# arneschneuing/DiffSBDD

Hardware: AMD Instinct MI355X
Metric: sampled ligands/sec (500-step DDPM, fullatom_cond) at 1/2/4/8 MI355X (higher is better)
Workload: dtype f32

## Files before the change

diffsbdd_amd/csrc/engine.hip:

```cpp
#include "../../include/diffsbdd_hip.h"

#include <cstdio>
#include <cstdlib>
#include <cstring>
#include <string>
#include <vector>

#include "common.h"
#include "ddpm.h"
#include "edge_mlp.h"
#include "edge_wave.h"
#include "edge_wave16.h"
#include "edge_splitk.h"
#include "graph.h"
#include "lig_head.h"
#include "molecule.h"
#include "node_chain.h"
#include "node_linear.h"
#include "train.h"

using namespace dsbdd;

static thread_local std::string g_err;
static int fail(int code, const std::string& msg) { g_err = msg; return code; }

#define HIP_TRY(expr)                                                              \
  do {                                                                             \
    hipError_t _e = (expr);                                                        \
    if (_e != hipSuccess)                                                          \
      return fail(DSBDD_ERR_LAUNCH, std::string(#expr) + ": " + hipGetErrorString(_e)); \
  } while (0)

struct StreamDevice {
  int prev = -1;
  bool switched = false;
  explicit StreamDevice(void* stream) {
    hipStream_t s = static_cast<hipStream_t>(stream);
    if (!s) return;
    hipDevice_t d = 0;
    int cur = 0;
    if (hipStreamGetDevice(s, &d) != hipSuccess || hipGetDevice(&cur) != hipSuccess) { (void)hipGetLastError(); return; }
    if ((int)d != cur) { prev = cur; switched = hipSetDevice((int)d) == hipSuccess; }
  }
  ~StreamDevice() { if (switched) (void)hipSetDevice(prev); }
  StreamDevice(const StreamDevice&) = delete;
  StreamDevice& operator=(const StreamDevice&) = delete;
};

static inline int pad4(int v) { return (v + 3) & ~3; }
static inline size_t al256(size_t v) { return (v + 255) & ~(size_t)255; }

struct dsbdd_engine {
  dsbdd_config cfg;
  std::vector<const float*> slots;
  bool has_weights = false;
  char* ws = nullptr;
  size_t ws_bytes = 0;
  int64_t cap_lig = 0, cap_poc = 0, cap_batch = 0, cap_edges = 0;
  int *node_batch, *lig_off, *poc_off, *deg, *row_ptr, *erow, *ecol;
  int *act_flag, *act_ptr, *act_list;
  float *ed0, *x, *x_in, *xagg, *mean, *h0, *enc_tmp, *h, *t1, *agg, *pq, *pqg, *hout, *w2tp;
  float *agg_head, *xagg_head;
  int *scan_tmp, *seg_base, *tile_ctr;
  int *erow2, *ecol2, *row_ptr2, *deg2, *scan_tmp2, *seg_base2;
  int *erow3, *ecol3, *row_ptr3, *deg3, *scan_tmp3, *seg_base3, *node_batch3, *lig_off3, *poc_off3, *twin;
  float *ed02, *ed03, *xframe, *aggB, *agg_headB;
  int* frame_rows;
  int *lvl, *seg_rows, *seg_edges, *node_base, *edge_base, *lvl_cnt, *lvl_end, *lvl_list, *row_ptrL, *erowL, *ecolL;
  float* ed0L;
  unsigned long long* lvl_stats = nullptr;
  bool lvl_stats_zeroed = false;
  int64_t cap_edgesL = 0;
  int prune = 1;
  int cone = 1;
  int64_t ghost_slots = 0;
  std::vector<int> plan_radius, plan_ghost;
  int plan_timed_level = kLevels - 1;
  bool frame = false;
  int64_t frame_nlig = 0, frame_npoc = 0, frame_batch = 0, frame_n3 = 0, frame_cap3 = 0;
  bool ghost_dirty = true;
  bool h0_pocket_valid = false;
  int64_t cap_tiles = 0;
  int64_t cap_tiles16 = 0;
  unsigned granule16 = 0;
  bool w2tp16_ready = false;
  unsigned splitk = 0;
  bool w2sk_ready = false;
  int emu = 0;
  bool w2e_ready = false;
  float *trace_h = nullptr, *trace_x = nullptr;
  int n_cu = 256;
  bool w2tp_ready = false;
  float* wchain = nullptr;
  bool wchain_ready = false;
  int chain = 1;
  int64_t chain_min_rows = 0;
  int fork_front = 0;
  hipStream_t side_stream = nullptr;
  hipEvent_t ev_fork = nullptr, ev_join = nullptr;
  int level_rows = 0;
  int fold_scan = 1;
  int lig_head = 1;
  int edge_bperm = 1;
  int profile = 0;
  int64_t prof_call = 0;
  bool time_now = false;
  std::vector<hipEvent_t> ev;
  size_t ev_used = 0;
  struct GraphEntry {
    std::vector<uint64_t> key;
    int seen = 0;
    hipGraph_t graph = nullptr;
    hipGraphExec_t exec = nullptr;
    std::vector<int> plan_radius, plan_ghost;
    int plan_timed_level = 0;
  };
  std::vector<GraphEntry> graphs;
  int use_graph = 1;
  int coord_split = 1;
  int node_group = 1;
  int edge_max_wg = 0;
  int64_t n_replay = 0, n_capture = 0, n_eager = 0;
  unsigned long long* ts_buf = nullptr;
  int ts_cap = 0, ts_next = 0;
  hipStream_t cap_stream = nullptr;
  void drop_graphs() {
    for (GraphEntry& g : graphs) {
      if (g.exec) (void)hipGraphExecDestroy(g.exec);
      if (g.graph) (void)hipGraphDestroy(g.graph);
    }
    graphs.clear();
  }
  ~dsbdd_engine() {
    for (hipEvent_t e : ev) (void)hipEventDestroy(e);
    drop_graphs();
    if (cap_stream) (void)hipStreamDestroy(cap_stream);
    if (side_stream) (void)hipStreamDestroy(side_stream);
    if (ev_fork) (void)hipEventDestroy(ev_fork);
    if (ev_join) (void)hipEventDestroy(ev_join);
  }
};

static int n_slots(const dsbdd_config& c) {
  return DSBDD_G_COUNT + c.n_layers * (c.inv_sublayers * DSBDD_GCL_COUNT + DSBDD_EQ_COUNT);
}
static int gcl_slot(const dsbdd_config& c, int block, int sub, int which) {
  return DSBDD_G_COUNT + block * (c.inv_sublayers * DSBDD_GCL_COUNT + DSBDD_EQ_COUNT) +
         sub * DSBDD_GCL_COUNT + which;
}
static int eq_slot(const dsbdd_config& c, int block, int which) {
  return DSBDD_G_COUNT + block * (c.inv_sublayers * DSBDD_GCL_COUNT + DSBDD_EQ_COUNT) +
         c.inv_sublayers * DSBDD_GCL_COUNT + which;
}

struct WsLayout {
  size_t off[72];
  size_t total;
};

static WsLayout carve(const dsbdd_config& c, int64_t nl, int64_t np, int64_t B, int64_t E) {
  const int64_t N = nl + np;
  const int H = c.hidden_nf, JP = pad4(c.joint_nf + 1);
  const int LE = pad4(2 * (c.atom_nf > c.residue_nf ? c.atom_nf : c.residue_nf));
  const int PQ = (c.reflection_equivariant ? 2 : 4) * H;
  const int64_t EL = 2 * E + 32 * kLevels * B;
  const int64_t NG = N + np;
  const int64_t T = EL / 32 + 2;
  size_t sizes[] = {
      (size_t)N * 4, (size_t)(B + 1) * 4, (size_t)(B + 1) * 4, (size_t)NG * 4, (size_t)(N + 1) * 4,
      (size_t)E * 4, (size_t)E * 4, (size_t)E * 4,
      (size_t)NG * 12, (size_t)N * 12, (size_t)N * 24, (size_t)B * 12,
      (size_t)N * JP * 4, (size_t)N * LE * 4,
      (size_t)NG * H * 4, (size_t)NG * H * 4, (size_t)NG * H * 4, (size_t)N * PQ * 4,
      (size_t)N * JP * 4,
      (size_t)N * 4, (size_t)(N + 1) * 4, (size_t)N * 4,
      (size_t)NG * 2 * H * 4,
      (size_t)c.n_layers * (c.inv_sublayers + 2) * H * H * 18 + 4096,
      (size_t)2 * T * H * 4, (size_t)2 * T * 2 * 16,
      (size_t)(N + 1) * 4, (size_t)(2 * B + 1) * 4, (size_t)kTileCtrInts * 4,
      (size_t)E * 4, (size_t)E * 4, (size_t)E * 4, (size_t)(N + 1) * 4, (size_t)N * 4,
      (size_t)(N + 1) * 4, (size_t)(2 * B + 1) * 4,
      (size_t)E * 4, (size_t)E * 4, (size_t)E * 4, (size_t)(N + 1) * 4, (size_t)N * 4,
      (size_t)(N + 1) * 4, (size_t)(2 * B + 1) * 4,
      (size_t)N * 4, (size_t)(B + 1) * 4, (size_t)(B + 1) * 4, (size_t)N * 4,
      (size_t)N * 12, (size_t)NG * H * 4, (size_t)T * H * 4,
      (size_t)N * 4, (size_t)kLevels * B * 4, (size_t)kLevels * B * 4,
      (size_t)(kLevels * B + 1) * 4, (size_t)(kLevels * B + 1) * 4, 64, 64,
      (size_t)NG * 4, (size_t)(NG + 1) * 4, (size_t)EL * 4, (size_t)EL * 4, (size_t)EL * 4,
      128, (size_t)N * 4,
      (size_t)c.n_layers * ((size_t)c.inv_sublayers * 5 * H * H + (size_t)H * PQ) * 4 + 4096};
  WsLayout L;
  size_t o = 0;
  const int n = sizeof(sizes) / sizeof(sizes[0]);
  for (int i = 0; i < n; ++i) { L.off[i] = o; o += al256(sizes[i] + 16); }
  L.total = o;
  return L;
}

static int build_edges_impl(hipStream_t s, const float* x, int n_lig, int N, int B, const dsbdd_config& c,
                            const int* node_batch, const int* lig_off, const int* poc_off, int* deg,
                            int* row_ptr, int* erow, int* ecol, float* ed0, int64_t cap, int* status,
                            int* act_flag = nullptr, int* scan_tmp = nullptr, int* seg_base = nullptr,
                            const EdgeList2* list2 = nullptr, int id_offset = 0, int* lvl = nullptr);

extern "C" {

int dsbdd_abi_version(void) { return DSBDD_ABI_VERSION; }
const char* dsbdd_last_error(void) { return g_err.c_str(); }

int dsbdd_engine_create(const dsbdd_config* cfg, dsbdd_engine** out) {
  if (!cfg || !out) return fail(DSBDD_ERR_ARG, "null argument");
  const int H = cfg->hidden_nf;
  if (!(H == 64 || H == 128 || H == 192 || H == 256))
    return fail(DSBDD_ERR_ARG, "hidden_nf must be one of 64, 128, 192, 256");
  if (cfg->n_layers < 1 || cfg->inv_sublayers < 1 || cfg->atom_nf < 1 || cfg->residue_nf < 1 ||
      cfg->joint_nf < 1 || cfg->edge_embedding_dim < 0)
    return fail(DSBDD_ERR_ARG, "bad layer/feature counts");
  if (!(cfg->normalization_factor > 0.f)) return fail(DSBDD_ERR_ARG, "normalization_factor must be > 0");
  dsbdd_engine* e = new dsbdd_engine();
  e->cfg = *cfg;
  e->slots.assign(n_slots(*cfg), nullptr);
  int dev = 0;
  hipDeviceProp_t prop;
  if (hipGetDevice(&dev) == hipSuccess && hipGetDeviceProperties(&prop, dev) == hipSuccess &&
      prop.multiProcessorCount > 0)
    e->n_cu = prop.multiProcessorCount;
  const char* ug = getenv("DSBDD_GRAPH");
  if (ug && atoi(ug) == 0) e->use_graph = 0;
  const char* bpe = getenv("DSBDD_EDGE_BPERM");
  if (bpe && atoi(bpe) == 0) e->edge_bperm = 0;
  const char* csp = getenv("DSBDD_COORD_SPLIT");
  if (csp && atoi(csp) == 0) e->coord_split = 0;
  const char* ngp = getenv("DSBDD_NODE_GROUP");
  if (ngp && atoi(ngp) == 0) e->node_group = 0;
  const char* prn = getenv("DSBDD_PRUNE");
  if (prn && atoi(prn) == 0) e->prune = 0;
  if (const char* lh = getenv("DSBDD_LIG_HEAD")) e->lig_head = atoi(lh) != 0;
  if (const char* fs = getenv("DSBDD_FOLD_SCAN")) e->fold_scan = atoi(fs) > 0 ? 1 : 0;
  if (const char* lr = getenv("DSBDD_LEVEL_ROWS")) e->level_rows = atoi(lr) != 0;
  if (const char* fk = getenv("DSBDD_FORK")) e->fork_front = atoi(fk) != 0;
  if (const char* g16 = getenv("DSBDD_GRANULE16")) e->granule16 = (unsigned)strtoul(g16, nullptr, 0);
  if (const char* sk = getenv("DSBDD_SPLITK")) e->splitk = (unsigned)strtoul(sk, nullptr, 0);
  if (const char* em = getenv("DSBDD_EMU")) { const int v = atoi(em); e->emu = (v == 6 || v == 9) ? v : 0; }
  const char* cn = getenv("DSBDD_CONE");
  if (cn) e->cone = atoi(cn) <= 0 ? 0 : (atoi(cn) >= 2 ? 2 : 1);
  const char* nch = getenv("DSBDD_NODE_CHAIN");
  if (nch && atoi(nch) == 0) e->chain = 0;
  const char* ncm = getenv("DSBDD_NODE_CHAIN_MIN_ROWS");
  if (ncm && atoi(ncm) >= 0) e->chain_min_rows = atoi(ncm);
  const char* mwg = getenv("DSBDD_EDGE_MAX_WG");
  if (mwg && atoi(mwg) > 0) e->edge_max_wg = atoi(mwg);
  *out = e;
  return DSBDD_OK;
}

void dsbdd_engine_destroy(dsbdd_engine* e) { delete e; }

int dsbdd_engine_weight_slots(const dsbdd_engine* e) { return e ? n_slots(e->cfg) : DSBDD_ERR_ARG; }

int dsbdd_engine_set_weights(dsbdd_engine* e, const float* const* slots_host, int n) {
  if (!e || !slots_host) return fail(DSBDD_ERR_ARG, "null argument");
  if (n != n_slots(e->cfg)) return fail(DSBDD_ERR_ARG, "wrong number of weight slots");
  const dsbdd_config& c = e->cfg;
  for (int i = 0; i < n; ++i) {
    const float* ptr = slots_host[i];
    bool optional = false;
    const int per = c.inv_sublayers * DSBDD_GCL_COUNT + DSBDD_EQ_COUNT;
    if (i >= DSBDD_G_COUNT) {
      const int r = (i - DSBDD_G_COUNT) % per;
      if (r < c.inv_sublayers * DSBDD_GCL_COUNT) {
        const int wch = r % DSBDD_GCL_COUNT;
        if (!c.attention && (wch == DSBDD_GCL_ATT_W || wch == DSBDD_GCL_ATT_B)) optional = true;
      } else {
        const int wch = r - c.inv_sublayers * DSBDD_GCL_COUNT;
        if (c.reflection_equivariant && wch >= DSBDD_EQ_X_WD && wch <= DSBDD_EQ_X_B2) optional = true;
      }
    }
    if (!ptr && !optional) return fail(DSBDD_ERR_ARG, "null weight slot " + std::to_string(i));
    if (ptr && (reinterpret_cast<uintptr_t>(ptr) & 15))
      return fail(DSBDD_ERR_ARG, "weight slot " + std::to_string(i) + " not 16-byte aligned");
    e->slots[i] = ptr;
  }
  e->drop_graphs();
  e->w2tp_ready = false;
  e->w2tp16_ready = false;
  e->w2sk_ready = false;
  e->w2e_ready = false;
  e->wchain_ready = false;
  e->h0_pocket_valid = false;
  e->has_weights = true;
  return DSBDD_OK;
}

size_t dsbdd_engine_workspace_bytes(const dsbdd_engine* e, int64_t nl, int64_t np, int64_t B,
                                    int64_t E) {
  if (!e || nl < 0 || np < 0 || B < 1 || E < 0) return 0;
  return carve(e->cfg, nl, np, B, E).total;
}

int dsbdd_engine_bind_workspace(dsbdd_engine* e, void* ws, size_t bytes, int64_t nl, int64_t np,
                                int64_t B, int64_t E) {
  if (!e || !ws) return fail(DSBDD_ERR_ARG, "null argument");
  if (reinterpret_cast<uintptr_t>(ws) & 255) return fail(DSBDD_ERR_ARG, "workspace must be 256-byte aligned");
  if ((nl + np) >= (1ll << 30) || E >= (1ll << 31) - 256) return fail(DSBDD_ERR_ARG, "problem too large for int32 indices");
  WsLayout L = carve(e->cfg, nl, np, B, E);
  if (bytes < L.total) return fail(DSBDD_ERR_CAPACITY, "workspace too small");
  char* b = static_cast<char*>(ws);
  e->drop_graphs();
  e->ws = b; e->ws_bytes = bytes;
  e->cap_lig = nl; e->cap_poc = np; e->cap_batch = B; e->cap_edges = E;
  e->node_batch = (int*)(b + L.off[0]); e->lig_off = (int*)(b + L.off[1]); e->poc_off = (int*)(b + L.off[2]);
  e->deg = (int*)(b + L.off[3]); e->row_ptr = (int*)(b + L.off[4]);
  e->erow = (int*)(b + L.off[5]); e->ecol = (int*)(b + L.off[6]); e->ed0 = (float*)(b + L.off[7]);
  e->x = (float*)(b + L.off[8]); e->x_in = (float*)(b + L.off[9]); e->xagg = (float*)(b + L.off[10]);
  e->mean = (float*)(b + L.off[11]); e->h0 = (float*)(b + L.off[12]); e->enc_tmp = (float*)(b + L.off[13]);
  e->h = (float*)(b + L.off[14]); e->t1 = (float*)(b + L.off[15]); e->agg = (float*)(b + L.off[16]);
  e->pq = (float*)(b + L.off[17]); e->hout = (float*)(b + L.off[18]);
  e->act_flag = (int*)(b + L.off[19]); e->act_ptr = (int*)(b + L.off[20]); e->act_list = (int*)(b + L.off[21]);
  e->pqg = (float*)(b + L.off[22]);
  e->w2tp = (float*)(b + L.off[23]);
// ... 548 lines not shown
    return (e->splitk && can_sk) ? reinterpret_cast<const float*>(reinterpret_cast<const char*>(e->w2tp) + n_w2 * H * H * 14) +
                                       ((size_t)blk * (c.inv_sublayers + 2) + which) * H * H
                                 : nullptr;
  };
  if (e->splitk && can_sk && !e->w2sk_ready) {
    for (int blk = 0; blk < c.n_layers; ++blk)
      for (int which = 0; which < c.inv_sublayers + 2; ++which) {
        const float* src = which < c.inv_sublayers ? W[gcl_slot(c, blk, which, DSBDD_GCL_E2_WT)]
                         : W[eq_slot(c, blk, which == c.inv_sublayers ? DSBDD_EQ_C_W2T : DSBDD_EQ_X_W2T)];
        if (!src) continue;
        hipLaunchKernelGGL(pack_w2sk_kernel, dim3((H * H + 255) / 256), dim3(256), 0, s, src,
                           const_cast<float*>(w2sk_of(blk, which)), H);
        HIP_TRY(hipGetLastError());
      }
    e->w2sk_ready = true;
  }
  if (e->emu && !e->w2e_ready) {
    for (int blk = 0; blk < c.n_layers; ++blk)
      for (int which = 0; which < c.inv_sublayers + 2; ++which) {
        const float* src = which < c.inv_sublayers ? W[gcl_slot(c, blk, which, DSBDD_GCL_E2_WT)]
                         : W[eq_slot(c, blk, which == c.inv_sublayers ? DSBDD_EQ_C_W2T : DSBDD_EQ_X_W2T)];
        if (!src) continue;
        hipLaunchKernelGGL(pack_w2e_kernel, dim3((H * H + 255) / 256), dim3(256), 0, s, src,
                           reinterpret_cast<unsigned short*>(const_cast<void*>(w2e_of(blk, which))), H);
        HIP_TRY(hipGetLastError());
      }
    e->w2e_ready = true;
  }
  if (e->granule16 && !e->w2tp16_ready) {
    for (int blk = 0; blk < c.n_layers; ++blk)
      for (int which = 0; which < c.inv_sublayers + 2; ++which) {
        const float* src = which < c.inv_sublayers ? W[gcl_slot(c, blk, which, DSBDD_GCL_E2_WT)]
                         : W[eq_slot(c, blk, which == c.inv_sublayers ? DSBDD_EQ_C_W2T : DSBDD_EQ_X_W2T)];
        if (!src) continue;
        hipLaunchKernelGGL(pack16_w2t_kernel, dim3((H * H + 255) / 256), dim3(256), 0, s, src,
                           const_cast<float*>(w2tp16_of(blk, which)), H);
        HIP_TRY(hipGetLastError());
      }
    e->w2tp16_ready = true;
  }
  if (bperm && !e->w2tp_ready) {
    for (int blk = 0; blk < c.n_layers; ++blk)
      for (int which = 0; which < c.inv_sublayers + 2; ++which) {
        const float* src = which < c.inv_sublayers ? W[gcl_slot(c, blk, which, DSBDD_GCL_E2_WT)]
                         : W[eq_slot(c, blk, which == c.inv_sublayers ? DSBDD_EQ_C_W2T : DSBDD_EQ_X_W2T)];
        if (!src) continue;
        hipLaunchKernelGGL(permute_w2t_kernel, dim3((H * H + 255) / 256), dim3(256), 0, s, src,
                           const_cast<float*>(w2tp_of(blk, which)), H);
        HIP_TRY(hipGetLastError());
      }
    e->w2tp_ready = true;
  }
  const bool use_chain = e->chain && (H == 256 || H == 192 || H == 128) && N >= e->chain_min_rows;
  const size_t chain_blk = (size_t)c.inv_sublayers * 5 * H * H + (size_t)H * PQ;
  auto chain_w = [&](int blk, int sub, int which) -> const float* {
    const float* base = e->wchain + (size_t)blk * chain_blk;
    if (which == 3) return base + (size_t)c.inv_sublayers * 5 * H * H;
    return base + (size_t)sub * 5 * H * H + (which == 0 ? 0 : (which == 1 ? 2 * H * H : 3 * H * H));
  };
  if (use_chain && !e->wchain_ready) {
    auto pack = [&](const float* WT, int ldw, int K, int Ncols, const float* dst) {
      hipLaunchKernelGGL(pack_b16_kernel, dim3((K * Ncols + 255) / 256), dim3(256), 0, s, WT, ldw, K, Ncols,
                         const_cast<float*>(dst));
    };
    for (int blk = 0; blk < c.n_layers; ++blk) {
      for (int sub = 0; sub < c.inv_sublayers; ++sub) {
        pack(W[gcl_slot(c, blk, sub, DSBDD_GCL_N1_WT)], H, 2 * H, H, chain_w(blk, sub, 0));
        pack(W[gcl_slot(c, blk, sub, DSBDD_GCL_N2_WT)], H, H, H, chain_w(blk, sub, 1));
        pack(W[gcl_slot(c, blk, sub, DSBDD_GCL_E1_WT)], 2 * H, H, 2 * H, chain_w(blk, sub, 2));
      }
      pack(W[eq_slot(c, blk, DSBDD_EQ_C1_WT)], PQ, H, PQ, chain_w(blk, 0, 3));
    }
    HIP_TRY(hipGetLastError());
    e->wchain_ready = true;
  }
  auto gcl_pq = [&](int blk, int sub) {
    NodeLinearArgs a{e->h, H, H, nullptr, 0, 0, W[gcl_slot(c, blk, sub, DSBDD_GCL_E1_WT)], 2 * H, nullptr,
                     nullptr, 0, e->pqg, 2 * H, (int)N, 2 * H, 0, nullptr, nullptr};
    const int g = blk * c.inv_sublayers + sub;
    rows_of(radius_of(g) + 1, g <= g_ghost_last && g > 0, a);
    return a;
  };
  bool pqg_ready = false, chained_pq = false, chained_coord = false;
  for (int blk = 0; blk < c.n_layers; ++blk) {
    if (n_mlp == 2 && (blk == 0 || !subset) && !(blk == 0 && mean_in_levels)) {
      hipLaunchKernelGGL(sample_mean_kernel, dim3(B), dim3(kThreads), 0, s, (const float*)e->x,
                         (const int*)e->lig_off, (const int*)e->poc_off, nlig, e->mean);
      HIP_TRY(hipGetLastError());
    }
    for (int sub = 0; sub < c.inv_sublayers; ++sub) {
      auto G = [&](int which) { return W[gcl_slot(c, blk, sub, which)]; };
      if (sub > 0 && chained_pq) pqg_ready = true;
      if (!pqg_ready) {
        const bool rows0 = split0 && blk == 0 && sub == 0;
        NodeLinearArgs grp0[2];
        if (rows0) {
          grp0[0] = gcl_pq(blk, sub);
          grp0[0].row_idx = act_rows; grp0[0].m_count = act_count; grp0[0].M = N;
          grp0[1] = gcl_pq(blk, sub);
          grp0[1].A1 = e->h + (size_t)N * H; grp0[1].C = e->pqg + (size_t)N * 2 * H; grp0[1].M = n_frame_rows;
          grp0[1].row_idx = nullptr; grp0[1].m_count = nullptr;
        }
        if (!(rows0 && launch_node_group(s, grp0, 2) == hipSuccess)) {
          (void)hipGetLastError();
          HIP_TRY(launch_node_linear(s, gcl_pq(blk, sub)));
          if (rows0) HIP_TRY(launch_node_linear(s, grp0[1]));
        }
      }
      pqg_ready = false;
      const int g = blk * c.inv_sublayers + sub;
      const int radius = radius_of(g);
      const bool ghost = g <= g_ghost_last;
      const bool all_rows = !prune || radius >= LV;
      const int64_t begin = ghost ? 0 : ghost_slots;
      EdgeArgs ea{};
      ea.erow = L_row + begin; ea.ecol = L_col + begin; ea.ed0 = L_d0 + begin;
      ea.e_count = !prune ? e_all : (ghost ? e->lvl_end + radius : e->lvl_end + kLevels + radius);
      ea.e_cap = L_cap - (int)begin; ea.wt_base = (int)(begin / 32); ea.x = e->x;
      ea.n_lig = nlig; ea.n_nodes = N + n_frame_rows; ea.ldpq = 2 * H;
      ea.mlp[0] = EdgeMlpW{e->pqg, e->pqg + H, G(DSBDD_GCL_E1_WD), G(DSBDD_GCL_E1_WD0), G(DSBDD_GCL_E1_TAB),
                           G(DSBDD_GCL_E2_WT), G(DSBDD_GCL_E2_B), w2tp_of(blk, sub), w2tp16_of(blk, sub), w2e_of(blk, sub),
                           w2sk_of(blk, sub)};
      ea.mlp[1] = ea.mlp[0];
      const bool g16 = ((e->granule16 >> (g & 15)) & 1u) && !(split0 && blk == 0 && sub == 0) && !e->emu;
      const bool gsk = ((e->splitk >> (g & 15)) & 1u) && can_sk;
      ea.att_w = G(DSBDD_GCL_ATT_W); ea.att_b = G(DSBDD_GCL_ATT_B); ea.attention = c.attention;
      ea.agg = e->agg; ea.agg_head = e->agg_head; ea.tile_ctr = e->tile_ctr;
      ea.norm_factor = c.normalization_factor;
      if (split0 && blk == 0 && sub == 0) {
        EdgeArgs a2 = ea;
        a2.erow = e->erow2; a2.ecol = e->ecol2; a2.ed0 = e->ed02; a2.e_count = e->row_ptr2 + N;
        a2.e_cap = (int)e->cap_edges; a2.wt_base = 0;
        EdgeArgs a3 = ea;
        a3.erow = e->erow3; a3.ecol = e->ecol3; a3.ed0 = e->ed03; a3.e_count = e->row_ptr3 + e->frame_n3;
        a3.agg = e->aggB; a3.agg_head = e->agg_headB; a3.e_cap = (int)e->cap_edges; a3.wt_base = 0;
        a2.erow_b = a3.erow; a2.ecol_b = a3.ecol; a2.ed0_b = a3.ed0; a2.e_count_b = a3.e_count; a2.e_cap_b = a3.e_cap;
        a2.wt_base_b = a3.wt_base; a2.agg_b = a3.agg; a2.agg_head_b = a3.agg_head;
        HIP_TRY(launch_edge(e, s, MODE_GCL, a2, edge_bound + ((e->frame_cap3 + 127) / 128) * 128, false, gsk));
        hipLaunchKernelGGL(agg_complete2_kernel, dim3((N + n_ghost + 3) / 4), dim3(kThreads), 0, s, e->agg,
                           (const float*)e->agg_head, (const int*)e->row_ptr2, (const int*)e->deg2,
                           (const float*)e->aggB, (const float*)e->agg_headB, (const int*)e->row_ptr3,
                           (const int*)e->deg3, (const int*)e->twin, N, nlig, N, H, cone ? n_ghost : 0, (int)e->cap_tiles - 1);
        HIP_TRY(hipGetLastError());
      } else {
        const bool timed = e->time_now && (all_rows || radius == e->plan_timed_level) && e->ev_used + 2 <= e->ev.size();
        if (timed) HIP_TRY(hipEventRecord(e->ev[e->ev_used], s));
        HIP_TRY(launch_edge(e, s, MODE_GCL, ea, L_bound, g16 && !gsk, gsk));
        if (timed) {
          HIP_TRY(hipEventRecord(e->ev[e->ev_used + 1], s));
          e->ev_used += 2;
        }
        const int n_rows = N + (ghost ? n_ghost : 0);
        hipLaunchKernelGGL(agg_complete_kernel, dim3((n_rows + 3) / 4), dim3(kThreads), 0, s, e->agg,
                           (const float*)e->agg_head, L_ptr, (const int*)e->deg, n_rows, H,
                           (int)((g16 && !gsk) ? e->cap_tiles16 : e->cap_tiles) - 1, (g16 && !gsk) ? 4 : 5);
        HIP_TRY(hipGetLastError());
      }
      NodeLinearArgs n1{e->h, H, H, e->agg, H, H, G(DSBDD_GCL_N1_WT), H, G(DSBDD_GCL_N1_B), nullptr, 0, e->t1, H,
                        (int)N, H, 1, nullptr, nullptr};
      NodeLinearArgs n2{e->t1, H, H, nullptr, 0, 0, G(DSBDD_GCL_N2_WT), H, G(DSBDD_GCL_N2_B), e->h, H, e->h, H,
                        (int)N, H, 0, nullptr, nullptr};
      rows_of(radius, ghost, n1); rows_of(radius, ghost, n2);
      chained_pq = false; chained_coord = false;
      bool fill_pq = false;
      if (use_chain) {
        NodeChainArgs ca{};
        ca.row_idx = n1.row_idx; ca.m_count = n1.m_count; ca.M = n1.M; ca.do_mlp = 1;
        ca.h = e->h; ca.agg = e->agg;
        ca.W1p = chain_w(blk, sub, 0); ca.b1 = G(DSBDD_GCL_N1_B);
        ca.W2p = chain_w(blk, sub, 1); ca.b2 = G(DSBDD_GCL_N2_B);
        const bool last_sub = sub + 1 == c.inv_sublayers;
        const int first = ghost ? n_ghost : 0;
        if (last_sub) {
          const int QW = n_mlp * H;
          const float* wc = chain_w(blk, 0, 3);
          if (!subset) {
            ca.proj[ca.n_proj++] = ChainProj{wc, e->pq, PQ, PQ, nullptr, 0};
            chained_coord = true;
          } else if (prune && n1.row_idx) {
            ca.proj[ca.n_proj++] = ChainProj{wc, e->pq, PQ, QW, act_count, first};
            ca.proj[ca.n_proj++] = ChainProj{wc + (size_t)(QW / 16) * (H / 16) * 256, e->pq + QW, PQ, QW,
                                             e->lvl_cnt + kLevels, first};
            chained_coord = true;
          }
        }
        const bool has_next = !last_sub || blk + 1 < c.n_layers;
        if (has_next) {
          const int nb = last_sub ? blk + 1 : blk, ns = last_sub ? 0 : sub + 1;
          const NodeLinearArgs nx = gcl_pq(nb, ns);
          const bool same_rows = nx.row_idx == n1.row_idx && nx.m_count == n1.m_count && nx.M == n1.M;
          if (same_rows || ghost) {
            ca.proj[ca.n_proj++] = ChainProj{chain_w(nb, ns, 2), e->pqg, 2 * H, 2 * H, nullptr, 0};
            chained_pq = true;
            fill_pq = ghost && !same_rows;
          }
        }
        HIP_TRY(launch_node_chain(s, ca, H, e->n_cu));
      } else {
        HIP_TRY(launch_node_linear(s, n1));
        HIP_TRY(launch_node_linear(s, n2));
      }
      if (ghost) {
        const int hi = radius_of(g + 1) + 1 < LV ? radius_of(g + 1) + 1 : LV;
        if (hi > radius) {
          hipLaunchKernelGGL(canon_fill_kernel, dim3((N - nlig + 3) / 4), dim3(kThreads), 0, s, e->h,
                             (const int*)e->lvl, (const int*)e->twin, nlig, N, N, radius, hi, H,
                             fill_pq ? e->pqg : (float*)nullptr, 2 * H);
          fill_pq = false;
          HIP_TRY(hipGetLastError());
        }
      }
    }
    {
      auto Q = [&](int which) { return W[eq_slot(c, blk, which)]; };
      const int QW = n_mlp * H;
      NodeLinearArgs grp[kMaxGroup];
      int ng = 0;
      if (!chained_coord) {
        if (subset) {
          grp[ng++] = NodeLinearArgs{e->h, H, H, nullptr, 0, 0, Q(DSBDD_EQ_C1_WT), PQ, nullptr, nullptr, 0, e->pq, PQ,
                                     (int)N, QW, 0, act_rows, act_count};
          grp[ng++] = NodeLinearArgs{e->h, H, H, nullptr, 0, 0, Q(DSBDD_EQ_C1_WT) + QW, PQ, nullptr, nullptr, 0,
                                     e->pq + QW, PQ, (int)n_lig, QW, 0, nullptr, nullptr};
        } else {
          grp[ng++] = NodeLinearArgs{e->h, H, H, nullptr, 0, 0, Q(DSBDD_EQ_C1_WT), PQ, nullptr, nullptr, 0, e->pq, PQ,
                                     (int)N, PQ, 0, nullptr, nullptr};
        }
      }
      const int n_coord = ng;
      const bool want_next = blk + 1 < c.n_layers && !chained_pq;
      if (chained_pq && blk + 1 < c.n_layers) pqg_ready = true;
      if (want_next && use_chain) {
        const NodeLinearArgs nx = gcl_pq(blk + 1, 0);
        NodeChainArgs ca{};
        ca.row_idx = nx.row_idx; ca.m_count = nx.m_count; ca.M = nx.M; ca.do_mlp = 0; ca.h = e->h;
        ca.n_proj = 1;
        ca.proj[0] = ChainProj{chain_w(blk + 1, 0, 2), e->pqg, 2 * H, 2 * H, nullptr, 0};
        HIP_TRY(launch_node_chain(s, ca, H, e->n_cu));
        pqg_ready = true;
      } else if (want_next) {
        grp[ng++] = gcl_pq(blk + 1, 0);
      }
      if (ng > 0) {
        if (e->node_group && launch_node_group(s, grp, ng) == hipSuccess) {
          if (ng > n_coord) pqg_ready = true;
        } else {
          (void)hipGetLastError();
          for (int i = 0; i < n_coord; ++i) HIP_TRY(launch_node_linear(s, grp[i]));
        }
      }
      chained_pq = false;
// ... 945 lines not shown
```

diffsbdd_amd/csrc/node_chain.h:

```cpp
#pragma once
#include "common.h"

namespace dsbdd {

typedef float f32x4 __attribute__((ext_vector_type(4)));

#ifdef DSBDD_CHAIN_TS
__device__ unsigned long long* g_chain_ts = nullptr;
__device__ __forceinline__ void chain_ts(int slot) {
  if (g_chain_ts && threadIdx.x == 0 && slot < 16) {
    g_chain_ts[blockIdx.x * 32 + slot] = __builtin_readcyclecounter();
    g_chain_ts[blockIdx.x * 32 + 16 + slot] = wall_clock64();
  }
}
#define CHAIN_TS(k) chain_ts(k)
#define CHAIN_NOTE(slot, v) do { if (g_chain_ts && threadIdx.x == 0) g_chain_ts[blockIdx.x * 32 + (slot)] = (unsigned long long)(v); } while (0)
#else
#define CHAIN_TS(k) do { } while (0)
#define CHAIN_NOTE(slot, v) do { } while (0)
#endif

constexpr int kChainThreads = 512;
constexpr int kChainRowsMax = 96;
constexpr int kChainChunkK = 64;
constexpr int kChainMaxProj = 3;

__global__ void pack_b16_kernel(const float* WT, int ldw, int K, int N, float* dst) {
  const int idx = blockIdx.x * blockDim.x + threadIdx.x;
  if (idx >= K * N) return;
  const int s = idx & 3, lane = (idx >> 2) & 63, rest = idx >> 8;
  const int g = rest % (K / 16), ct = rest / (K / 16);
  dst[idx] = WT[(size_t)(16 * g + 4 * (lane >> 4) + s) * ldw + 16 * ct + (lane & 15)];
}

struct ChainProj {
  const float* Wp;
  float* C; int ldc;
  int N;
  const int* count;
  int first;
};

struct NodeChainArgs {
  const int* row_idx;
  const int* m_count;
  int M;
  int do_mlp;
  float* h;
  const float* agg;
  const float* W1p; const float* b1;
  const float* W2p; const float* b2;
  int n_proj;
  ChainProj proj[kChainMaxProj];
};

__device__ __forceinline__ f32x4 mfma16(float a, float b, f32x4 c) {
  return __builtin_amdgcn_mfma_f32_16x16x4f32(a, b, c, 0, 0, 0);
}

template <int RT, int CT>
__device__ __forceinline__ void chain_mfma_group(f32x4 (&acc)[RT][CT], const float4 (&wv)[CT], const float4 (&xv)[RT]) {
  __builtin_amdgcn_s_setprio(1);
#pragma unroll
  for (int s = 0; s < 4; ++s)
#pragma unroll
    for (int rt = 0; rt < RT; ++rt)
#pragma unroll
      for (int t = 0; t < CT; ++t) {
        const float a = s == 0 ? wv[t].x : (s == 1 ? wv[t].y : (s == 2 ? wv[t].z : wv[t].w));
        const float b = s == 0 ? xv[rt].x : (s == 1 ? xv[rt].y : (s == 2 ? xv[rt].z : xv[rt].w));
        acc[rt][t] = mfma16(a, b, acc[rt][t]);
      }
  __builtin_amdgcn_s_setprio(0);
}

template <int RT, int CT, bool CHUNKED, class XOf, class Hook>
__device__ __forceinline__ void chain_kloop(f32x4 (&acc)[RT][CT], XOf&& x_of, const float* wp, size_t wstride, int NG,
                                            Hook&& next_chunk) {
  float4 w0[CT], w1[CT], x0[RT], x1[RT];
  auto load = [&](int g, float4 (&wv)[CT], float4 (&xv)[RT]) {
#ifdef DSBDD_DIAG_CHAIN_NOW
    if (g == 0)
#endif
#pragma unroll
    for (int t = 0; t < CT; ++t) wv[t] = ld4(wp + t * wstride + (size_t)g * 256);
    const float* xs = x_of(g);
#ifdef DSBDD_DIAG_CHAIN_NOX
    if (g == 0)
#endif
#pragma unroll
    for (int rt = 0; rt < RT; ++rt) xv[rt] = *reinterpret_cast<const float4*>(xs + 64 * rt);
  };
  if (!CHUNKED) {
    load(0, w0, x0);
#pragma unroll 1
    for (int g = 0; g + 2 < NG; g += 2) {
      load(g + 1, w1, x1);
      chain_mfma_group<RT, CT>(acc, w0, x0);
      load(g + 2, w0, x0);
      chain_mfma_group<RT, CT>(acc, w1, x1);
    }
    load(NG - 1, w1, x1);
    chain_mfma_group<RT, CT>(acc, w0, x0);
    chain_mfma_group<RT, CT>(acc, w1, x1);
  } else {
#pragma unroll 1
    for (int g = 0; g < NG; g += 4) {
      next_chunk(g >> 2);
      load(g, w0, x0);
      load(g + 1, w1, x1);
      chain_mfma_group<RT, CT>(acc, w0, x0);
      load(g + 2, w0, x0);
      chain_mfma_group<RT, CT>(acc, w1, x1);
      load(g + 3, w1, x1);
      chain_mfma_group<RT, CT>(acc, w0, x0);
      chain_mfma_group<RT, CT>(acc, w1, x1);
      __syncthreads();
    }
  }
}

#ifndef DSBDD_CHAIN_WHOLE
#define DSBDD_CHAIN_WHOLE 1
#endif
#ifndef DSBDD_CHAIN_PRE
#define DSBDD_CHAIN_PRE 1
#endif

template <int H, int RT>
__device__ __forceinline__ void chain_range(const NodeChainArgs& p, const int r0, const int M, float* smem,
                                            const int* pcount) {
  constexpr int R16 = 16 * RT;
  constexpr int kLdsFloats = kChainRowsMax * H + 2 * (kChainChunkK / 4) * kChainRowsMax * 4;
  constexpr bool WHOLE = DSBDD_CHAIN_WHOLE && R16 * 3 * H <= kLdsFloats;
  float* sPanel = smem;
  float* sChunk = smem + R16 * H;
  constexpr int CTW = H >= 192 ? 2 : 1;
  constexpr int NG = H / 16;
  constexpr int CHP = kChainChunkK / 4;
  static_assert(H % 64 == 0 && H <= 256, "hidden_nf");
  const int t = threadIdx.x, lane = t & 63, w = t >> 6;
  const int i = lane & 15, kq = lane >> 4;
  auto phys = [&](int logical) {
    const int c = logical < M ? logical : M - 1;
    return p.row_idx ? p.row_idx[c] : c;
  };
  const float* xs = sPanel + (kq * R16 + i) * 4;
  const bool col_active = w * CTW * 16 < H;

  auto dma_panels = [&](const float* src, int k0, int n_panels, float* dst) {
    const int ra = phys(r0 + lane), rb = phys(r0 + 64 + lane);
    for (int q = w; q < n_panels; q += 8) {
      if (R16 >= 64 || lane < R16)
        __builtin_amdgcn_global_load_lds((const __attribute__((address_space(1))) void*)(src + (size_t)ra * H + k0 + 4 * q),
                                         (__attribute__((address_space(3))) void*)(dst + q * R16 * 4), 16, 0, 0);
      if (R16 > 64 && lane < R16 - 64)
        __builtin_amdgcn_global_load_lds((const __attribute__((address_space(1))) void*)(src + (size_t)rb * H + k0 + 4 * q),
                                         (__attribute__((address_space(3))) void*)(dst + (q * R16 + 64) * 4), 16, 0, 0);
    }
  };

  int rowp[RT];
#pragma unroll
  for (int rt = 0; rt < RT; ++rt) rowp[rt] = phys(r0 + 16 * rt + i);

  CHAIN_TS(1);
  CHAIN_NOTE(8, r0); CHAIN_NOTE(9, R16);
  int n_pass = 0;
  (void)n_pass;
  if (p.do_mlp) {
    {
      f32x4 acc[RT][CTW];
#pragma unroll
      for (int rt = 0; rt < RT; ++rt)
#pragma unroll
        for (int c = 0; c < CTW; ++c) acc[rt][c] = f32x4{0.f, 0.f, 0.f, 0.f};
      constexpr int NCH = 2 * H / kChainChunkK;
      const float* wp = p.W1p + ((size_t)(w * CTW) * (2 * H / 16) * 64 + lane) * 4;
      const size_t wstride = (size_t)(2 * H / 16) * 256;
      auto chunk_src = [&](int c) { return c * kChainChunkK < H ? p.h : p.agg; };
      auto chunk_k0 = [&](int c) { return c * kChainChunkK < H ? c * kChainChunkK : c * kChainChunkK - H; };
      if constexpr (WHOLE) {
        dma_panels(p.h, 0, H / 4, sChunk);
        dma_panels(p.agg, 0, H / 4, sChunk + (H / 4) * R16 * 4);
        __syncthreads();
        const float* xb = sChunk + (kq * R16 + i) * 4;
        auto x_all = [&](int g) { return xb + (size_t)g * 16 * R16; };
        auto no_hook = [](int) {};
        if (col_active) chain_kloop<RT, CTW, false>(acc, x_all, wp, wstride, 2 * H / 16, no_hook);
        __syncthreads();
      } else {
        constexpr int CB = CHP * R16 * 4;
        dma_panels(chunk_src(0), chunk_k0(0), CHP, sChunk);
        __syncthreads();
        const float* xb = sChunk + (kq * R16 + i) * 4;
        auto x_of = [&](int g) { return xb + ((g >> 2) & 1) * CB + (g & 3) * 16 * R16; };
        auto next_chunk = [&](int c) {
          if (c + 1 < NCH) dma_panels(chunk_src(c + 1), chunk_k0(c + 1), CHP, sChunk + ((c + 1) & 1) * CB);
        };
        if (col_active) {
          chain_kloop<RT, CTW, true>(acc, x_of, wp, wstride, 2 * H / 16, next_chunk);
        } else {
#pragma unroll 1
          for (int c = 0; c < NCH; ++c) {
            next_chunk(c);
            __syncthreads();
          }
        }
      }
      CHAIN_TS(2);
#pragma unroll
      for (int c = 0; c < (col_active ? CTW : 0); ++c) {
        const int col = 16 * (w * CTW + c) + 4 * kq;
        const float4 bv = ld4(p.b1 + col);
#pragma unroll
        for (int rt = 0; rt < RT; ++rt) {
          float4 v;
          v.x = silu(acc[rt][c][0] + bv.x); v.y = silu(acc[rt][c][1] + bv.y);
          v.z = silu(acc[rt][c][2] + bv.z); v.w = silu(acc[rt][c][3] + bv.w);
          *reinterpret_cast<float4*>(sPanel + ((col >> 2) * R16 + 16 * rt + i) * 4) = v;
        }
      }
      __syncthreads();
      CHAIN_TS(3);
#pragma unroll
      for (int rt = 0; rt < RT; ++rt)
#pragma unroll
        for (int c = 0; c < CTW; ++c) acc[rt][c] = f32x4{0.f, 0.f, 0.f, 0.f};
      auto x_panel = [&](int g) { return xs + (size_t)g * 16 * R16; };
      auto no_hook = [](int) {};
      constexpr bool PRE = DSBDD_CHAIN_PRE && RT <= 4;
      float4 hn[RT][CTW];
      auto load_res = [&]() {
#pragma unroll
        for (int c = 0; c < (col_active ? CTW : 0); ++c)
#pragma unroll
          for (int rt = 0; rt < RT; ++rt) hn[rt][c] = ld4(p.h + (size_t)rowp[rt] * H + 16 * (w * CTW + c) + 4 * kq);
      };
      if (PRE) load_res();
      if (col_active)
        chain_kloop<RT, CTW, false>(acc, x_panel, p.W2p + ((size_t)(w * CTW) * NG * 64 + lane) * 4, (size_t)NG * 256, NG, no_hook);
      if (!PRE) load_res();
      CHAIN_TS(4);
#pragma unroll
      for (int c = 0; c < (col_active ? CTW : 0); ++c) {
        const int col = 16 * (w * CTW + c) + 4 * kq;
        const float4 bv = ld4(p.b2 + col);
#pragma unroll
        for (int rt = 0; rt < RT; ++rt) {
          float4 v = hn[rt][c];
          v.x += acc[rt][c][0] + bv.x; v.y += acc[rt][c][1] + bv.y;
          v.z += acc[rt][c][2] + bv.z; v.w += acc[rt][c][3] + bv.w;
          hn[rt][c] = v;
          if (r0 + 16 * rt + i < M) *reinterpret_cast<float4*>(p.h + (size_t)rowp[rt] * H + col) = v;
        }
      }
      if (p.n_proj > 0) {
        __syncthreads();
#pragma unroll
        for (int c = 0; c < (col_active ? CTW : 0); ++c) {
          const int col = 16 * (w * CTW + c) + 4 * kq;
#pragma unroll
          for (int rt = 0; rt < RT; ++rt) *reinterpret_cast<float4*>(sPanel + ((col >> 2) * R16 + 16 * rt + i) * 4) = hn[rt][c];
        }
        __syncthreads();
      }
    }
  } else if (p.n_proj > 0) {
    dma_panels(p.h, 0, H / 4, sPanel);
    __syncthreads();
  }

  CHAIN_TS(5);
  for (int q = 0; q < p.n_proj; ++q) {
    const ChainProj& pj = p.proj[q];
    const int lo = pj.first, cnt = pj.first + pcount[q];
// ... 218 lines not shown
```

Before: 38.59.

## Fold edge aggregation completion into the node chain kernel prologue

Removes the separate agg_complete/agg_complete2 kernel launches when the node chain path is used with H=256. Each chain workgroup now sums the per-tile partial aggregation heads for its own rows before DMA-loading agg into LDS. This cuts one launch and one global round trip of agg per sublayer. In exchange it adds serial work and extra loads inside the chain kernel's prologue, which could lengthen its critical path.

```diff
diff --git a/diffsbdd_amd/csrc/engine.hip b/diffsbdd_amd/csrc/engine.hip
--- a/diffsbdd_amd/csrc/engine.hip
+++ b/diffsbdd_amd/csrc/engine.hip
@@ -102,6 +102,7 @@
   int fold_scan = 1;
   int lig_head = 1;
   int edge_bperm = 1;
+  int glue_fold = 1;
   int profile = 0;
   int64_t prof_call = 0;
   bool time_now = false;
@@ -236,6 +237,7 @@
   const char* prn = getenv("DSBDD_PRUNE");
   if (prn && atoi(prn) == 0) e->prune = 0;
   if (const char* lh = getenv("DSBDD_LIG_HEAD")) e->lig_head = atoi(lh) != 0;
+  if (const char* gf = getenv("DSBDD_GLUE_FOLD")) e->glue_fold = atoi(gf) != 0;
   if (const char* fs = getenv("DSBDD_FOLD_SCAN")) e->fold_scan = atoi(fs) > 0 ? 1 : 0;
   if (const char* lr = getenv("DSBDD_LEVEL_ROWS")) e->level_rows = atoi(lr) != 0;
   if (const char* fk = getenv("DSBDD_FORK")) e->fork_front = atoi(fk) != 0;
@@ -950,6 +952,7 @@
     return a;
   };
   bool pqg_ready = false, chained_pq = false, chained_coord = false;
+  const bool fold_agg = e->glue_fold && use_chain && H == 256;
   for (int blk = 0; blk < c.n_layers; ++blk) {
     if (n_mlp == 2 && (blk == 0 || !subset) && !(blk == 0 && mean_in_levels)) {
       hipLaunchKernelGGL(sample_mean_kernel, dim3(B), dim3(kThreads), 0, s, (const float*)e->x,
@@ -977,6 +980,7 @@
       }
       pqg_ready = false;
       const int g = blk * c.inv_sublayers + sub;
+      ChainAgg cagg{};
       const int radius = radius_of(g);
       const bool ghost = g <= g_ghost_last;
       const bool all_rows = !prune || radius >= LV;
@@ -1005,11 +1009,14 @@
         a2.erow_b = a3.erow; a2.ecol_b = a3.ecol; a2.ed0_b = a3.ed0; a2.e_count_b = a3.e_count; a2.e_cap_b = a3.e_cap;
         a2.wt_base_b = a3.wt_base; a2.agg_b = a3.agg; a2.agg_head_b = a3.agg_head;
         HIP_TRY(launch_edge(e, s, MODE_GCL, a2, edge_bound + ((e->frame_cap3 + 127) / 128) * 128, false, gsk));
-        hipLaunchKernelGGL(agg_complete2_kernel, dim3((N + n_ghost + 3) / 4), dim3(kThreads), 0, s, e->agg,
-                           (const float*)e->agg_head, (const int*)e->row_ptr2, (const int*)e->deg2,
-                           (const float*)e->aggB, (const float*)e->agg_headB, (const int*)e->row_ptr3,
-                           (const int*)e->deg3, (const int*)e->twin, N, nlig, N, H, cone ? n_ghost : 0, (int)e->cap_tiles - 1);
-        HIP_TRY(hipGetLastError());
+        cagg = ChainAgg{2, e->agg_head, e->row_ptr2, e->deg2, (int)N, (int)e->cap_tiles - 1, 5,
+                        e->aggB, e->agg_headB, e->row_ptr3, e->deg3, e->twin, (int)N, (int)nlig, cone ? (int)n_ghost : 0};
+        if (!fold_agg) {
+          hipLaunchKernelGGL(agg_complete2_kernel, dim3((N + n_ghost + 3) / 4), dim3(kThreads), 0, s, e->agg,
+                             cagg.head, cagg.row_ptr, cagg.deg, cagg.agg_b, cagg.head_b, cagg.row_ptr_b, cagg.deg_b,
+                             cagg.twin_local, cagg.twin_base, cagg.n_lig, cagg.n_rows, H, cagg.n_ghost, cagg.max_tile);
+          HIP_TRY(hipGetLastError());
+        }
       } else {
         const bool timed = e->time_now && (all_rows || radius == e->plan_timed_level) && e->ev_used + 2 <= e->ev.size();
         if (timed) HIP_TRY(hipEventRecord(e->ev[e->ev_used], s));
@@ -1019,10 +1026,14 @@
           e->ev_used += 2;
         }
         const int n_rows = N + (ghost ? n_ghost : 0);
-        hipLaunchKernelGGL(agg_complete_kernel, dim3((n_rows + 3) / 4), dim3(kThreads), 0, s, e->agg,
-                           (const float*)e->agg_head, L_ptr, (const int*)e->deg, n_rows, H,
-                           (int)((g16 && !gsk) ? e->cap_tiles16 : e->cap_tiles) - 1, (g16 && !gsk) ? 4 : 5);
-        HIP_TRY(hipGetLastError());
+        cagg = ChainAgg{};
+        cagg.mode = 1; cagg.head = e->agg_head; cagg.row_ptr = L_ptr; cagg.deg = e->deg; cagg.n_rows = n_rows;
+        cagg.max_tile = (int)((g16 && !gsk) ? e->cap_tiles16 : e->cap_tiles) - 1; cagg.shift = (g16 && !gsk) ? 4 : 5;
+        if (!fold_agg) {
+          hipLaunchKernelGGL(agg_complete_kernel, dim3((n_rows + 3) / 4), dim3(kThreads), 0, s, e->agg, cagg.head,
+                             cagg.row_ptr, cagg.deg, n_rows, H, cagg.max_tile, cagg.shift);
+          HIP_TRY(hipGetLastError());
+        }
       }
       NodeLinearArgs n1{e->h, H, H, e->agg, H, H, G(DSBDD_GCL_N1_WT), H, G(DSBDD_GCL_N1_B), nullptr, 0, e->t1, H,
                         (int)N, H, 1, nullptr, nullptr};
@@ -1035,6 +1046,7 @@
         NodeChainArgs ca{};
         ca.row_idx = n1.row_idx; ca.m_count = n1.m_count; ca.M = n1.M; ca.do_mlp = 1;
         ca.h = e->h; ca.agg = e->agg;
+        if (fold_agg) ca.cagg = cagg;
         ca.W1p = chain_w(blk, sub, 0); ca.b1 = G(DSBDD_GCL_N1_B);
         ca.W2p = chain_w(blk, sub, 1); ca.b2 = G(DSBDD_GCL_N2_B);
         const bool last_sub = sub + 1 == c.inv_sublayers;
diff --git a/diffsbdd_amd/csrc/node_chain.h b/diffsbdd_amd/csrc/node_chain.h
--- a/diffsbdd_amd/csrc/node_chain.h
+++ b/diffsbdd_amd/csrc/node_chain.h
@@ -41,13 +41,23 @@
   int first;
 };
 
+struct ChainAgg {
+  int mode;
+  const float* head;
+  const int* row_ptr; const int* deg;
+  int n_rows, max_tile, shift;
+  const float* agg_b; const float* head_b; const int* row_ptr_b; const int* deg_b; const int* twin_local;
+  int twin_base, n_lig, n_ghost;
+};
+
 struct NodeChainArgs {
   const int* row_idx;
   const int* m_count;
   int M;
   int do_mlp;
   float* h;
-  const float* agg;
+  float* agg;
+  ChainAgg cagg;
   const float* W1p; const float* b1;
   const float* W2p; const float* b2;
   int n_proj;
@@ -160,6 +170,69 @@
     }
   };
 
+  auto complete_agg = [&]() {
+    const ChainAgg& a = p.cagg;
+    const int wu = __builtin_amdgcn_readfirstlane(w);
+    const int k = 4 * lane;
+    const float4 zero = make_float4(0.f, 0.f, 0.f, 0.f);
+    constexpr int NR = R16 / 8, CB = NR < 6 ? NR : 6;
+#pragma unroll
+    for (int jb = 0; jb < NR; jb += CB) {
+      int row[CB], ta0[CB], ta1[CB], tb0[CB], tb1[CB], tw[CB];
+      bool act[CB], has_a[CB], has_b[CB], put[CB];
+      int na = 0, nb = 0;
+#pragma unroll
+      for (int j = 0; j < CB; ++j) {
+        const int lr = r0 + wu + 8 * (jb + j);
+        row[j] = phys(lr < M ? lr : M - 1);
+        act[j] = jb + j < NR && lr < M && row[j] < a.n_rows + (a.mode == 2 ? a.n_ghost : 0);
+        const bool ghost = a.mode == 2 && row[j] >= a.n_rows;
+        const int d = (act[j] && !ghost) ? a.deg[row[j]] : 0, s = (act[j] && !ghost) ? a.row_ptr[row[j]] : 0;
+        ta0[j] = s >> a.shift; ta1[j] = min((s + d - 1) >> a.shift, a.max_tile);
+        has_a[j] = d > 0;
+        int db = 0, sb = 0;
+        tw[j] = 0;
+        if (act[j] && a.mode == 2 && row[j] >= a.n_lig) {
+          const int tl = ghost ? row[j] - a.n_rows : a.twin_local[row[j] - a.n_lig];
+          db = a.deg_b[tl]; sb = a.row_ptr_b[tl]; tw[j] = a.twin_base + tl;
+        }
+        tb0[j] = sb >> 5; tb1[j] = min((sb + db - 1) >> 5, a.max_tile);
+        has_b[j] = db > 0;
+        put[j] = act[j] && !(has_a[j] && ta1[j] == ta0[j] && (a.mode == 1 || !has_b[j]));
+        if (put[j] && has_a[j]) na = max(na, ta1[j] - ta0[j]);
+        if (put[j] && has_b[j]) nb = max(nb, tb1[j] - tb0[j]);
+      }
+      float4 va[CB], vb[CB], hv[CB];
+#pragma unroll
+      for (int j = 0; j < CB; ++j) {
+        va[j] = (put[j] && has_a[j] && k < H) ? ld4(p.agg + (size_t)row[j] * H + k) : zero;
+        vb[j] = (put[j] && has_b[j] && k < H) ? ld4(a.agg_b + (size_t)tw[j] * H + k) : zero;
+      }
+      for (int st = 1; st <= na; ++st) {
+#pragma unroll
+        for (int j = 0; j < CB; ++j)
+          hv[j] = (put[j] && has_a[j] && ta0[j] + st <= ta1[j] && k < H) ? ld4(a.head + (size_t)(ta0[j] + st) * H + k) : zero;
+#pragma unroll
+        for (int j = 0; j < CB; ++j)
+          if (put[j] && has_a[j] && ta0[j] + st <= ta1[j]) { va[j].x += hv[j].x; va[j].y += hv[j].y; va[j].z += hv[j].z; va[j].w += hv[j].w; }
+      }
+      for (int st = 1; st <= nb; ++st) {
+#pragma unroll
+        for (int j = 0; j < CB; ++j)
+          hv[j] = (put[j] && has_b[j] && tb0[j] + st <= tb1[j] && k < H) ? ld4(a.head_b + (size_t)(tb0[j] + st) * H + k) : zero;
+#pragma unroll
+        for (int j = 0; j < CB; ++j)
+          if (put[j] && has_b[j] && tb0[j] + st <= tb1[j]) { vb[j].x += hv[j].x; vb[j].y += hv[j].y; vb[j].z += hv[j].z; vb[j].w += hv[j].w; }
+      }
+#pragma unroll
+      for (int j = 0; j < CB; ++j) {
+        float4 v = va[j];
+        if (has_b[j]) { v.x += vb[j].x; v.y += vb[j].y; v.z += vb[j].z; v.w += vb[j].w; }
+        if (put[j] && k < H) *reinterpret_cast<float4*>(p.agg + (size_t)row[j] * H + k) = v;
+      }
+    }
+  };
+
   int rowp[RT];
 #pragma unroll
   for (int rt = 0; rt < RT; ++rt) rowp[rt] = phys(r0 + 16 * rt + i);
@@ -182,6 +255,10 @@
       auto chunk_k0 = [&](int c) { return c * kChainChunkK < H ? c * kChainChunkK : c * kChainChunkK - H; };
       if constexpr (WHOLE) {
         dma_panels(p.h, 0, H / 4, sChunk);
+        if (p.cagg.mode) {
+          complete_agg();
+          __syncthreads();
+        }
         dma_panels(p.agg, 0, H / 4, sChunk + (H / 4) * R16 * 4);
         __syncthreads();
         const float* xb = sChunk + (kq * R16 + i) * 4;
@@ -192,6 +269,8 @@
       } else {
         constexpr int CB = CHP * R16 * 4;
         dma_panels(chunk_src(0), chunk_k0(0), CHP, sChunk);
+        static_assert(kChainChunkK <= H, "chunk 0 must not read agg");
+        if (p.cagg.mode) complete_agg();
         __syncthreads();
         const float* xb = sChunk + (kq * R16 + i) * 4;
         auto x_of = [&](int g) { return xb + ((g >> 2) & 1) * CB + (g & 3) * 16 * R16; };
```

After: 38.76, median of 6. No clear change (+0.4%).
